# GEM3D/pressurePoissonSolver

Hardware: AMD Instinct MI355X
Metric: V-cycle lattice-site updates/sec, 512^3 3D Poisson (higher is better)
Workload: dtype f64; 1 GPU; apps/3d/steady-equivalent: 512^3 uniform, 4096 patches of 32^3, 5 levels, V(1,1), smoother=rbgs, Dirichlet, f ~ U(-1,1) splitmix64(0x5EED + patch id); workload_key=3d:u512:p32:rbgs, parallelism=patch-sharded x1 (Morton ranges), exchange=none, levels=5, smoother=rbgs

## Files before the change

include/te_hip.h:

```cpp
#ifndef TE_HIP_H
#define TE_HIP_H
#include <stddef.h>
#include <stdint.h>
#ifdef __cplusplus
extern "C" {
#endif

#define TE_OK 0
#define TE_EINVAL -1
#define TE_EHIP -2
#define TE_ESTATE -3
#define TE_EIO -4
#define TE_EUNSUPPORTED -5
#define TE_ENOMEM -6

typedef struct te_mesh te_mesh;
typedef struct te_hier te_hier;
typedef struct te_gmg  te_gmg;
typedef struct te_vec  te_vec;

const char *te_last_error(void);
const char *te_version(void);

int te_mesh_read(const char *path, int dim, te_mesh **out);
// ... 104 lines not shown
                double tol, int *iterations, double *rel_resid);
int te_gmg_release_workspace(te_gmg *g);

int te_prolong_quadratic(te_gmg *g, int fine_level, const te_vec *coarse, te_vec *fine);
int te_fmg(te_gmg *g, const te_cycle_opts *o, const te_vec *f, const te_vec *bdata, te_vec *u, int cycles, double *rel_resid);

int te_patch_indicator(te_gmg *g, int level, const te_vec *u, double *out_host);
int te_vec_regrid(te_gmg *src, const te_vec *u_src, te_gmg *dst, te_vec *u_dst);
int te_faces_regrid(te_gmg *src, const te_vec *U_src, te_gmg *dst, te_vec *U_dst);

int te_gmg_set_option(te_gmg *g, const char *name, const char *value);

enum { TE_SLABS_STENCIL = 0, TE_SLABS_SWEEP = 1 };
int te_gmg_slab_count(const te_gmg *g, int level, int kind, int *zs);

typedef int (*te_exchange_fn)(void *user, int tag, const double *send, double *recv, int npeers,
                              const int32_t *peers, const int64_t *send_off,
                              const int64_t *send_cnt, const int64_t *recv_off,
                              const int64_t *recv_cnt, void *stream);
int te_gmg_set_exchange(te_gmg *g, te_exchange_fn fn, void *user);
int te_rccl_unique_id(const char *libpath, char *id128);
int te_gmg_use_rccl(te_gmg *g, const char *libpath, const char *id128, int rank, int nranks);
typedef int (*te_allreduce_fn)(void *user, double *vals, int n, int op);
int te_gmg_set_allreduce(te_gmg *g, te_allreduce_fn fn, void *user);
int te_gmg_verify_schedule(te_gmg *g, const te_cycle_opts *o);
int te_gmg_autotune(te_gmg *g, const te_cycle_opts *o, int reps, double *best_ms, char *report, int report_len);
int te_gmg_use_push(te_gmg *g, int enable);
int te_gmg_push_failed(te_gmg *g);

int te_gmg_set_patch_bcgs(te_gmg *g, double tol, int max_it);
// ... 56 lines not shown
```

pressurepoissonsolver_amd/capi.py:

```python
import ctypes as C
import os

import numpy as np

_HERE = os.path.dirname(os.path.abspath(__file__))
LIB_PATH = os.environ.get("TE_HIP_LIB_PATH") or os.path.join(_HERE, "libte_hip.so")


class TeError(RuntimeError):

    def __init__(self, code, msg):
        super().__init__(f"te_hip error {code}: {msg}")
        self.code = code


class TeLibraryMissing(ImportError):
    pass


TE_OK, TE_EINVAL, TE_EHIP, TE_ESTATE, TE_EIO, TE_EUNSUPPORTED, TE_ENOMEM = 0, -1, -2, -3, -4, -5, -6
SMOOTH_PATCH_SOLVE, SMOOTH_JACOBI, SMOOTH_RBGS, SMOOTH_PATCH_BCGS = 0, 1, 2, 3
PROBLEM_TRIG, PROBLEM_GAUSS, PROBLEM_RANDOM = 0, 1, 2
SCHUR_PREC_NONE, SCHUR_PREC_CHEB = 0, 1
INTERP_DIRECT, INTERP_LINEAR = 0, 1
# ... 93 lines not shown
    "te_prolong_add": (_I, [_P, _I, _P, _P]),
    "te_prolong_linear_add": (_I, [_P, _I, _P, _P]),
    "te_prolong_quadratic": (_I, [_P, _I, _P, _P]),
    "te_boundary_restrict": (_I, [_P, _I, _P, _P]),
    "te_fmg": (_I, [_P, _P, _P, _P, _P, _I, _PD]),
    "te_patch_indicator": (_I, [_P, _I, _P, _P]),
    "te_vec_regrid": (_I, [_P, _P, _P, _P]),
    "te_faces_regrid": (_I, [_P, _P, _P, _P]),
    "te_gmg_set_interpolator": (_I, [_P, _I]),
    "te_gmg_interpolator": (_I, [_P]),
    "te_vcycle": (_I, [_P, C.POINTER(CycleOpts), _P, _P]),
    "te_bicgstab": (_I, [_P, C.POINTER(CycleOpts), _P, _P, _I, _D, C.POINTER(_I), _PD]),
    "te_gmg_release_workspace": (_I, [_P]),
    "te_gmg_set_option": (_I, [_P, C.c_char_p, C.c_char_p]),
    "te_gmg_slab_count": (_I, [_P, _I, _I, _P]),
    "te_gmg_set_exchange": (_I, [_P, EXCHANGE_FN, _P]),
    "te_rccl_unique_id": (_I, [C.c_char_p, C.c_char_p]),
    "te_gmg_use_rccl": (_I, [_P, C.c_char_p, C.c_char_p, _I, _I]),
    "te_gmg_set_allreduce": (_I, [_P, ALLREDUCE_FN, _P]),
    "te_gmg_verify_schedule": (_I, [_P, C.POINTER(CycleOpts)]),
    "te_gmg_autotune": (_I, [_P, C.POINTER(CycleOpts), _I, _PD, C.c_char_p, _I]),
    "te_gmg_comm_info": (_I, [_P, C.POINTER(_I), C.POINTER(_I)]),
    "te_gmg_use_push": (_I, [_P, _I]),
    "te_gmg_push_failed": (_I, [_P]),
    "te_gmg_set_patch_bcgs": (_I, [_P, _D, _I]),
    "te_gmg_patch_bcgs_iterations": (_I, [_P, _I, _P]),
    "te_gmg_exchange_selftest": (_I, [_P, _I]),
    "te_gmg_watchdog_selftest": (_I, [_P, _D]),
    "te_gmg_setup_ms": (_I, [_P, _PD, _I]),
    "te_gmg_profile": (_I, [_P, _I]),
# ... 478 lines not shown
        return its[:n_local]

    def comm_info(self):
        a, b = C.c_int(), C.c_int()
        check(lib().te_gmg_comm_info(self.h, C.byref(a), C.byref(b)))
        return a.value, b.value

    def set_option(self, name, value="1"):
        check(lib().te_gmg_set_option(self.h, name.encode(), None if value is None else str(value).encode()))

    def slab_count(self, level, kind=0):
        zs = C.c_int()
        check(lib().te_gmg_slab_count(self.h, level, kind, C.byref(zs)))
        return zs.value

    def release_workspace(self):
        check(lib().te_gmg_release_workspace(self.h))

    def set_allreduce(self, fn):
        def cb(user, vals, n, op):
            try:
                out = fn([vals[i] for i in range(n)], op)
                for i in range(n):
                    vals[i] = out[i]
                return 0
            except Exception:
                import traceback
                traceback.print_exc()
                return 1
        self._ar = ALLREDUCE_FN(cb)
# ... 84 lines not shown
```

pressurepoissonsolver_amd/csrc/gmg_core.hip:

```cpp
#include "gmg_internal.hpp"

namespace tei
{
const char *kclassName[KC_COUNT] = {"stencil_apply", "stencil_resid", "stencil_jacobi", "stencil_rbgs",
                                    "cf_ghost", "restrict", "prolong_add", "patch_rhs", "dst_axis",
                                    "vecop", "reduce", "pack", "exchange", "stencil_rbgs_zero", "resid_restrict", "patch_solve_mfma", "stencil_rbgs_prolong",
                                    "stencil_rbgs_slabs", "stencil_slabs", "patch_solve_3pass", "rbgs_zero_resid_restrict",
                                    "restrict_fixup", "rbgs_resweep_prolong", "rbgs_zero_resid_restrict_faces",
                                    "rbgs_resweep_prolong_fcorr", "rbgs_zero_resid_restrict_faces_fcorr", "fcorr_gather", "patch_solve_mfma_faces",
                                    "bicg_update", "bicg_s", "bicg_p", "stencil_apply_dot", "patch_bcgs", "gradient", "divergence", "project", "prolong_linear", "prolong_quadratic", "boundary_restrict",
                                    "indicator", "regrid", "regrid_faces",
                                    "apply_coef", "resid_coef", "jacobi_coef", "rbgs_coef", "faces_restrict"};
const char *optName[O_COUNT] = {"TE_2D_SIMPLE", "TE_2D_NO_MFMA", "TE_2D_NO_PF", "TE_2D_NO_MR_FUSE", "TE_2D_TPB", "TE_NO_FUSE2", "TE_NO_FUSE3",
                                "TE_NO_FUSE3_CF", "TE_NO_CFP", "TE_NO_XF", "TE_NO_FCORR", "TE_NO_FCORR_CF", "TE_NO_OVERLAP",
                                "TE_OVERLAP_MIN", "TE_NO_PS_FACES", "TE_PS_MODE", "TE_PS_SLOW", "TE_RBGS_NOSLAB", "TE_ZS_FORCE", "TE_NO_ZS8",
                                "TE_RESWEEP_V", "TE_EXCHANGE_TIMEOUT", "TE_NO_VERIFY", "TE_RCCL_LOOPBACK", "TE_NO_BICG_FUSE", "TE_POST_EXCHANGE", "TE_REPL_BLOCKS", "TE_PACK_FACES", "TE_OVERLAP_MODE", "TE_PUSH_TIMEOUT", "TE_NO_BICG_XF", "TE_PUSH_FAULT", "TE_2D_NO_FOLD", "TE_2D_NO_SYM", "TE_PUSH_NONFATAL", "TE_PS_NO_HALF", "TE_PS_HALF_MAX", "TE_NO_RS6_CF", "TE_NO_RS6_FIXUP", "TE_SCHUR_FULL", "TE_ZS_PIN"};

void drainEvents(te_gmg *g)
{
	if (g->ev_used == 0) return;
	(void) hipStreamSynchronize(g->stream);
	for (size_t i = 0; i < g->ev_used; i++) {
		float ms = 0;
		if (g->ev_pool[i].valid && hipEventElapsedTime(&ms, g->ev_pool[i].a, g->ev_pool[i].b) == hipSuccess) {
			g->calls[g->ev_pool[i].kc]++;
			g->total_ms[g->ev_pool[i].kc] += ms;
		}
	}
	g->ev_used = 0;
}

// ... 46 lines not shown
	L->prolong_fusable = T.prolong_fusable, L->prolong_fusable_cf = T.prolong_fusable_cf, L->has_copy = T.has_copy;
	L->repl_up = T.repl_up, L->repl_direct = T.repl_direct, L->post_exchange_free = T.post_exchange_free;

	const size_t P1 = (size_t) std::max(T.P, 1), nf = T.nf;
	const bool   fused3d = (D == 3 && T.fuse2_ok && T.P > 0);
	if ((rc = L->send_faces.upload(T.send_faces)) || (rc = L->sendbuf.alloc((size_t) std::max(T.nremote, 1) * nf))
	    || (rc = L->f6off.upload(T.f6off)) || (rc = L->order.upload(T.order)))
		return rc;
	if (D == 3 && ((rc = L->xfbuf[0].alloc(P1 * 2 * nf)) || (rc = L->xfbuf[1].alloc(P1 * 2 * nf)) || (rc = L->f6buf.alloc(P1 * 6 * nf))))
		return rc;
	if (fused3d && li > 0) {
		if ((rc = L->fcorr.alloc((size_t) T.P * 4 * nf))) return rc;
		HIPCHK(hipMemset(L->fcorr.p, 0, sizeof(double) * L->fcorr.n));
	}
	if (fused3d && (rc = L->rs6.alloc((size_t) T.P * 6 * nf / 4))) return rc;
	if ((rc = L->geom_starts.upload(T.geom_starts)) || (rc = L->geom_h.upload(T.geom_h)) || (rc = L->node_ids.upload(T.node_ids))
	    || (rc = L->cellvol.upload(T.cellvol)) || (rc = L->face_kind_patch.upload(T.face_kind_patch))
	    || (rc = L->face_kind.upload(T.face_kind)) || (rc = L->face_src.upload(T.face_src)) || (rc = L->face_kadj.upload(T.face_kadj))
	    || (rc = L->rh2.upload(T.rh2)) || (rc = L->cf_desc.upload(T.cf_desc)) || (rc = L->cf_slots.upload(T.cf_slots))
	    || (rc = L->ghost.alloc((size_t) std::max(T.nslots, 1) * nf)))
		return rc;
	if ((rc = L->matfrag.upload(T.matfrag)) || (rc = L->matsym.upload(T.matsym)) || (rc = L->matsT.upload(T.matsT))
	    || (rc = L->psinv.upload(T.psinv)) || (rc = L->psitab.upload(T.psitab)) || (rc = L->ps_list.upload(T.ps_list))
	    || (rc = L->mat2sym.upload(T.mat2sym)) || (rc = L->ps2_list.upload(T.ps2_list))
	    || (rc = L->corr.alloc(P1 * 2 * D * nf)) || (rc = L->plan.upload(T.plan)) || (rc = L->mats.upload(T.mats))
	    || (rc = L->lam.upload(T.lam)) || (rc = L->zero_mode.upload(T.zero_mode)))
		return rc;
	if (T.coarser
	    && ((D == 2 && T.fuse2_ok && (rc = L->e4buf.alloc(P1 * 4 * n))) || (rc = L->slot_parent.upload(T.slot_parent))
	        || (rc = L->slot_orth.upload(T.slot_orth)) || (rc = L->bc_desc.upload(T.bc_desc)) || (rc = L->cbase.upload(T.cbase))
	        || (rc = L->parent.upload(T.parent)) || (rc = L->orth.upload(T.orth)) || (rc = L->child.upload(T.child))
	        || (rc = L->copy.upload(T.copy)) || (rc = L->up_desc.upload(T.up_desc)) || (rc = L->down_desc.upload(T.down_desc))
	        || (rc = L->up_off.upload(T.up_off)) || (rc = L->down_off.upload(T.down_off))
	        || (rc = L->upbuf.alloc((size_t) std::max<int64_t>(T.up_total, 1)))
	        || (rc = L->downbuf.alloc((size_t) std::max<int64_t>(T.down_total, 1)))))
		return rc;
	g->levels.push_back(std::move(L));
	return TE_OK;
}

int newVec(te_gmg *g, int level, te_vec **out)
{
	LevelHost &L = *g->levels[level];
	auto       v = new te_vec;
	v->g         = g;
// ... 484 lines not shown
}

int te_gmg_slab_count(const te_gmg *g, int level, int kind, int *zs)
{
	return guarded([&]() -> int {
			if (!g || !zs || level < 0 || level >= (int) g->levels.size() || (kind != TE_SLABS_STENCIL && kind != TE_SLABS_SWEEP))
				return te::fail(TE_EINVAL, "te_gmg_slab_count: bad argument");
			const LevelHost &L = *g->levels[level];
			if (L.dim != 3)
				*zs = 1;
			else
				*zs = kind == TE_SLABS_STENCIL ? stencilSlabCount(L.n, L.P, slabSwitches(g)) : rbgsSlabCount(L.n, L.P, slabSwitches(g));
			return TE_OK;
	});
}
}
```

pressurepoissonsolver_amd/csrc/gmg_cycle.hip:

```cpp
#include "gmg_internal.hpp"

namespace tei
{
int smoothOnce(te_gmg *g, int level, const te_vec *f, te_vec *u, int smoother, double omega, bool zero_guess = false, bool faces_only = false)
{
	if (g->coef_on) return coefSmoothOnce(g, level, f, u, smoother, omega);
	LevelHost &L = *g->levels[level];
	int        rc;
	const bool xfok = (L.dim == 3 && g->in_cycle);
	switch (smoother) {
		case TE_SMOOTH_PATCH_SOLVE: {
			bool swapped = false;
			rc           = patchSolve(g, L, f->d, u->d, {zero_guess, nullptr, faces_only}, &swapped);
			if (rc == TE_OK && swapped) swapData(u, L.t.get());
			return rc;
		}
		case TE_SMOOTH_JACOBI:
			L.xf_valid_for = nullptr;
			rc = launchStencil<MODE_JACOBI>(g, L, u->d, f->d, L.t->d, omega);
			if (rc) return rc;
			swapData(u, L.t.get());
			return TE_OK;
		case TE_SMOOTH_RBGS:
			rc = launchRbgs(g, L, u->d, f->d, L.t->d, zero_guess, nullptr, xfok ? xfFor(L, u->d) : nullptr,
			                xfok ? L.xfbuf[L.xf_cur ^ 1].p : nullptr);
			if (rc) return rc;
			if (xfok) xfProduced(L, L.t->d);
			swapData(u, L.t.get());
			return TE_OK;
		case TE_SMOOTH_PATCH_BCGS:
			L.xf_valid_for = nullptr;
			return patchBcgs2d(g, L, f->d, u->d, L.t->d);
		default: return te::fail(TE_EINVAL, "te_smooth: unknown smoother");
	}
}

struct CycleScope {
	te_gmg *g;
	void    forget() const { for (auto &L : g->levels) L->xf_valid_for = nullptr, L->ps_faces = false; }
	explicit CycleScope(te_gmg *g_) : g(g_)
	{
		forget();
		g->in_cycle = !g->cfg.has(O_NO_XF);
	}
	~CycleScope()
	{
		g->in_cycle = false;
		forget();
	}
};

int visit(te_gmg *g, const te_cycle_opts *o, int l, const te_vec *f, te_vec *u, bool u_zero)
{
	const int  nl       = (int) g->levels.size();
	const bool coarsest = (l == nl - 1);
	LevelHost &L        = *g->levels[l];
	int        rc;
	g->cur_level        = l;
	const bool drct = g->interp == TE_INTERP_DIRECT;
	const double *fcorr_in = (L.f_has_corr && L.fcorr.p) ? L.fcorr.p : nullptr;
	L.f_has_corr           = false;
	const Fold2DHost fold_in = L.fold_pending;
	L.fold_pending           = Fold2DHost();
	if (fold_in.fine && coarsest) return te::fail(TE_ESTATE, "te_vcycle: folded ghost terms without a reader");
	const PendingRhs *pend = (l == 0) ? g->pending_rhs : nullptr;
	if (l == 0) g->pending_rhs = nullptr;
	auto formRhs = [&]() -> int {
		if (!pend) return TE_OK;
		const PendingRhs &r = *pend;
		pend                = nullptr;
		if (r.n2 == 0 || g->recording) return TE_OK;
		Timed      t(g, r.kind == 1 ? KC_BICG_S : KC_BICG_P, r.n2 * 2);
		const dim3 grid(gridFor(r.n2, 256, 1 << 30));
// ... 8 lines not shown
	};
	auto       materialise = [&]() -> int {
        if (!u_zero) return TE_OK;
        u_zero         = false;
        L.xf_valid_for = nullptr;
        return vecop<VOP_SET>(u, nullptr, nullptr, 0.0, 0.0, 0.0);
	};
	const double *pending_prolong = nullptr;
	bool          u_unstored      = false;
	int           next_sweeps     = 0;
	auto smooth = [&](int sweeps, bool at_coarsest, bool final_call = false) -> int {
		int sm = o->smoother;
		if (at_coarsest && o->exact_coarse && L.P_global == 1) sm = TE_SMOOTH_PATCH_SOLVE;
		for (int i = 0; i < sweeps; i++) {
			int r;
			if (pending_prolong) {
				const double *c = pending_prolong;
				pending_prolong = nullptr;
				const bool last = final_call && i == sweeps - 1 && !(l == 0 && g->keep_final_xf);
				if (sm == TE_SMOOTH_PATCH_SOLVE) {
					bool swapped = false;
					if ((r = patchSolve(g, L, f->d, u->d, {false, c, false, !last}, &swapped))) return r;
					if (swapped) swapData(u, L.t.get());
					continue;
				}
				double *xo = last ? nullptr : L.xfbuf[L.xf_cur ^ 1].p;
				if (u_unstored) {
					u_unstored = false;
					if ((r = resweepProlong(g, L, f->d, L.t->d, c, xo, fcorr_in))) return r;
				} else if ((r = launchRbgs(g, L, u->d, f->d, L.t->d, false, c, xfFor(L, u->d), xo))) {
					return r;
				}
				if (xo)
					xfProduced(L, L.t->d);
				else
					L.xf_valid_for = nullptr;
				swapData(u, L.t.get());
				continue;
			}
			if (u_zero && ((L.dim == 3 && (sm == TE_SMOOTH_RBGS || sm == TE_SMOOTH_PATCH_SOLVE)) || (L.lds2d && sm == TE_SMOOTH_RBGS)
			               || (L.dim == 2 && sm == TE_SMOOTH_PATCH_SOLVE))) {
				u_zero = false;
				r      = smoothOnce(g, l, f, u, sm, o->omega, true);
			} else {
// ... 83 lines not shown
		if ((rc = smoothOnce(g, l, f, u, TE_SMOOTH_PATCH_SOLVE, o->omega, true, faces_only))) return rc;
		if ((rc = interfaceResidRestrict(g, L, u->d, xfFor(L, u->d), C.f->d, C.f->n))) return rc;
		have_coarse_f = true;
	} else if (o->fuse >= 2 && u_zero && o->pre_sweeps == 1 && o->smoother == TE_SMOOTH_PATCH_SOLVE && ps2dResidFusable(g, L) && !fold_in.fine) {
		if ((rc = formRhs())) return rc;
		u_zero = false;
		if ((rc = smoothOnce(g, l, f, u, TE_SMOOTH_PATCH_SOLVE, o->omega, true))) return rc;
		if ((rc = interfaceResidRestrict2d(g, L, u->d, C.f->d, C.f->n))) return rc;
		have_coarse_f = true;
	} else if (fcorr_in || fold_in.fine) {
		return te::fail(TE_ESTATE, "te_vcycle: exported ghost terms without a reader");
	} else if ((rc = formRhs()) || (rc = smooth(o->pre_sweeps, false))) {
		return rc;
	}
	next_sweeps = (o->cycle_type == 1) ? o->mid_sweeps : o->post_sweeps;
	if ((rc = descend())) return rc;
	if (o->cycle_type == 1) {
		if ((rc = smooth(o->mid_sweeps, false))) return rc;
		next_sweeps = o->post_sweeps;
		if ((rc = descend())) return rc;
	}
	return smooth(o->post_sweeps, false, true);
}

static uint64_t mix64(uint64_t h, uint64_t v)
{
	h ^= v + 0x9E3779B97F4A7C15ull + (h << 6) + (h >> 2);
	h *= 0xBF58476D1CE4E5B9ull;
	return h ^ (h >> 31);
}

// ... 466 lines not shown
```

pressurepoissonsolver_amd/csrc/gmg_fused3d.hip:

```cpp
#include "gmg_ghosts3d.hpp"

namespace tei
{
template <int N>
int zeroSweepResidN(te_gmg *g, LevelHost &L, const double *f, double *out, double *coarse, double *xf_out, bool store_u,
                    double *fcorr_out, const double *fcorr_in, const PendingRhs *fs)
{
	RestrictDst rd = restrictDst(L, coarse);
	const bool export_rs6 = L.rs6.p && !store_u
	                        && (fcorr_out ? (L.prolong_fusable || !g->cfg.has(O_NO_RS6_CF))
	                                      : (L.Pc > 0 || L.n_up > 0) && !fcorr_in && !g->cfg.has(O_NO_RS6_FIXUP));
	rd.rs6                = export_rs6 ? L.rs6.p : nullptr;
	int rc;
	if (L.P > 0) {
		Timed      t(g, store_u ? KC_ZERO_RESID : (fcorr_in ? KC_ZERO_RESID_FACES_FCORR : KC_ZERO_RESID_FACES), (size_t) L.P * L.nc, true);
		if (!store_u) L.f6_tab = L.f6off.p != nullptr && !g->cfg.has(O_PACK_FACES);
		LevelDev   D = L.dev();
		const dim3 grid = slabGrid(L.P), blk(Tile3<N>::TPB);
		if (store_u) {
			D.xf_out = xf_out;
			launchT(t, (k_rbgs_zero_resid3d<N, true>), grid, blk, 0, g->stream, D, f, out, rd, FSrc());
		} else {
			D.f6_out = L.f6buf.p;
			D.fcorr  = fcorr_in;
// ... 35 lines not shown
	} else if (L.P > 0) {
		Timed    t(g, KC_FIXUP, (size_t) L.P * 6 * L.nf);
		LevelDev D = L.dev();
		if (store_u)
			D.xf = xf_out;
		else
			D.f6 = L.f6buf.p;
		hipLaunchKernelGGL((k_restrict_fixup3d<N, false>), dim3(L.P), dim3(256), 0, g->stream, D, out, rd);
	}
	if ((rc = shipRestricted<N>(g, L, coarse))) return rc;
	HIPCHK(hipGetLastError());
	return TE_OK;
}

template <int N>
int resweepProlongN(te_gmg *g, LevelHost &L, const double *f, double *out, const double *prolong_from, double *xf_out, const double *fcorr_in)
{
	ProlongSrc ps      = prolongSrc(L, prolong_from);
	const bool refined = L.ncf > 0 || L.has_copy;
	const int v = resweepVariant(fcorr_in != nullptr, refined, L.index, (size_t) L.P * L.nc * sizeof(double), g->resweep_pin);
	if (!v) return te::fail(TE_ESTATE, "resweepProlong: exported ghost terms on a refined level");
	auto launch = [&](LevelDev D) {
		if (D.count == 0) return;
		Timed t(g, fcorr_in ? KC_RESWEEP_FCORR : KC_RESWEEP, (size_t) D.count * L.nc, true);
		D.f6    = L.f6buf.p;
		D.fcorr = fcorr_in;
		const dim3 grid = slabGrid(D.count), blk(Tile3<N>::TPB);
		if (refined) {
			if (v == 59)
				launchT(t, (k_rbgs_resweep_prolong3d<N, 59, false, true>), grid, blk, 0, g->stream, D, f, out, ps);
			else
				launchT(t, (k_rbgs_resweep_prolong3d<N, 27, false, true>), grid, blk, 0, g->stream, D, f, out, ps);
		} else if (v == 3) {
			launchT(t, (k_rbgs_resweep_prolong3d<N, 3, true>), grid, blk, 0, g->stream, D, f, out, ps);
// ... 10 lines not shown
		ps.gorth      = L.slot_orth.p;
		L.ghost_has_v = false;
		LevelDev D    = L.dev();
		D.xf_out      = xf_out;
		launch(D);
		HIPCHK(hipGetLastError());
		return TE_OK;
	}
	int rc = withGhosts<N>(g, L, {nullptr, L.f6buf.p, &ps}, launch, nullptr, xf_out);
	if (rc) return rc;
	HIPCHK(hipGetLastError());
	return TE_OK;
}

int resweepProlong(te_gmg *g, LevelHost &L, const double *f, double *out, const double *prolong_from, double *xf_out,
                   const double *fcorr_in)
{
	if (L.dim == 2) return resweepProlong2d(g, L, f, out, prolong_from);
	return dispatchN(L.n, [&](auto n) { return resweepProlongN<decltype(n)::value>(g, L, f, out, prolong_from, xf_out, fcorr_in); });
}

template <int N> int interfaceResidRestrictN(te_gmg *g, LevelHost &L, const double *u, const double *xf, double *coarse, size_t coarse_n)
{
	RestrictDst rd = restrictDst(L, coarse);
	int rc;
	if ((rc = prepareGhosts<N>(g, L, {u, L.ps_faces ? L.f6buf.p : nullptr}))) return rc;
	{
		Timed t(g, KC_VECOP, coarse_n);
		if (L.repl_up && L.repl_direct && !g->cfg.has(O_REPL_BLOCKS) && !L.tx_direct.empty()) {
			if (L.tx_direct.send_cnt[0] > 0)
				HIPCHK(hipMemsetAsync(coarse + L.tx_direct.send_off[0], 0, sizeof(double) * (size_t) L.tx_direct.send_cnt[0], g->stream));
		} else
			HIPCHK(hipMemsetAsync(coarse, 0, sizeof(double) * coarse_n, g->stream));
		if (L.n_up > 0) HIPCHK(hipMemsetAsync(L.upbuf.p, 0, sizeof(double) * L.upbuf.n, g->stream));
// ... 29 lines not shown
```

pressurepoissonsolver_amd/csrc/gmg_internal.hpp:

```cpp
#pragma once
#include "capi_common.hpp"
#include "dispatch.hpp"
#include "level_tables.hpp"
#include <hip/hip_ext.h>
#include <rccl/rccl.h>
#include "kernels3d.hpp"
#include "march3d.hpp"
#include "kernels2d.hpp"
#include "patchsolve32.hpp"
#include "patchsolve32_sym.hpp"
#include "patchsolve16.hpp"
#include "initkernels.hpp"
#include "bckernels.hpp"
#include "pushkernels.hpp"
#include <algorithm>
#include <array>
#include <atomic>
#include <chrono>
#include <cmath>
#include <cstdio>
#include <cstring>
#include <dlfcn.h>
#include <map>
#include <memory>
// ... 36 lines not shown
	KC_PS_MFMA_FACES,
	KC_BICG_UPDATE, KC_BICG_S, KC_BICG_P, KC_APPLY_DOT,
	KC_PATCH_BCGS,
	KC_GRADIENT, KC_DIVERGENCE, KC_PROJECT,
	KC_PROLONG_LINEAR,
	KC_PROLONG_QUADRATIC, KC_BOUNDARY_RESTRICT,
	KC_INDICATOR, KC_REGRID,
	KC_FACE_REGRID,
	KC_APPLY_COEF, KC_RESID_COEF, KC_JACOBI_COEF, KC_RBGS_COEF, KC_FACES_RESTRICT, KC_COUNT
};
extern const char *kclassName[KC_COUNT];

enum Opt : int {
	O_2D_SIMPLE, O_2D_NO_MFMA, O_2D_NO_PF, O_2D_NO_MR_FUSE, O_2D_TPB, O_NO_FUSE2, O_NO_FUSE3, O_NO_FUSE3_CF, O_NO_CFP, O_NO_XF,
	O_NO_FCORR, O_NO_FCORR_CF, O_NO_OVERLAP, O_OVERLAP_MIN, O_NO_PS_FACES, O_PS_MODE, O_PS_SLOW, O_RBGS_NOSLAB,
	O_ZS_FORCE, O_NO_ZS8, O_RESWEEP_V, O_EXCHANGE_TIMEOUT, O_NO_VERIFY, O_RCCL_LOOPBACK, O_NO_BICG_FUSE, O_POST_EXCHANGE, O_REPL_BLOCKS, O_PACK_FACES, O_OVERLAP_MODE, O_PUSH_TIMEOUT, O_NO_BICG_XF, O_PUSH_FAULT, O_2D_NO_FOLD, O_2D_NO_SYM, O_PUSH_NONFATAL, O_PS_NO_HALF, O_PS_HALF_MAX, O_NO_RS6_CF, O_NO_RS6_FIXUP, O_SCHUR_FULL, O_ZS_PIN, O_COUNT
};
extern const char *optName[O_COUNT];
inline bool optStructural(int o) { return o == O_2D_SIMPLE || o == O_NO_CFP || o == O_2D_NO_MR_FUSE || o == O_NO_OVERLAP || o == O_EXCHANGE_TIMEOUT; }
struct Cfg {
	bool        on[O_COUNT] = {};
	std::string val[O_COUNT];
	void        set(int o, const char *v)
	{
		on[o]  = v != nullptr;
		val[o] = v ? v : "";
	}
	void fromEnv();
	bool        has(int o) const { return on[o]; }
	const char *str(int o) const { return on[o] ? val[o].c_str() : nullptr; }
	int         num(int o, int dflt) const { return on[o] ? atoi(val[o].c_str()) : dflt; }
// ... 57 lines not shown
	bool   fuse2_ok = false;
	size_t nc = 0, nf = 0;
	DevBuf<int32_t> face_kind, face_src;
	DevBuf<int32_t> face_kind_patch;
	DevBuf<double>  face_kadj, rh2, ghost;
	int             nslots = 0;
	int             ncf = 0;
	DevBuf<int32_t> cf_desc, cf_slots;
	ExPlan          fx;
	int             nremote = 0;
	DevBuf<int32_t> send_faces;
	DevBuf<double>  sendbuf;
	int             Pc = 0;
	DevBuf<int32_t> parent, orth, child, copy;
	DevBuf<int64_t> cbase;
	ExPlan          tx_up, tx_down;
	int             n_up = 0, n_down = 0;
	bool            repl_up = false;
	DevBuf<int32_t> bc_desc;
	DevBuf<int32_t> up_desc, down_desc;
	DevBuf<int64_t> up_off, down_off;
	DevBuf<double>  upbuf, downbuf;
	DevBuf<int32_t> plan, zero_mode;
	DevBuf<int32_t> bcgs_its;
	DevBuf<double>  mats, lam, corr;
	DevBuf<double>  matsT;
	DevBuf<double>  matfrag;
	DevBuf<double>  matsym;
	DevBuf<double>  psinv;
	DevBuf<int32_t> psitab;
// ... 379 lines not shown
		if (idx < 0) return;
		auto &w = g->wd;
		std::lock_guard<std::mutex> lk(w.mu);
		w.batch     = -1;
		auto &sl    = w.slot[idx % te_gmg::Watchdog::RING];
		sl.recorded = (hipEventRecord(sl.ev, g->stream) == hipSuccess);
	}
};

template <int MODE> int launchStencil(te_gmg *g, LevelHost &L, const double *u, const double *f, double *out, double omega,
                                      RestrictDst rd = RestrictDst(), const double *xf_in = nullptr, int redmode = RED_NONE,
                                      const double *red_a = nullptr, int *red_items = nullptr, bool patch_op = false);
extern template int launchStencil<MODE_APPLY>(te_gmg *, LevelHost &, const double *, const double *, double *, double, RestrictDst, const double *, int, const double *, int *, bool);
extern template int launchStencil<MODE_RESID>(te_gmg *, LevelHost &, const double *, const double *, double *, double, RestrictDst, const double *, int, const double *, int *, bool);
extern template int launchStencil<MODE_JACOBI>(te_gmg *, LevelHost &, const double *, const double *, double *, double, RestrictDst, const double *, int, const double *, int *, bool);
int resweepProlong(te_gmg *g, LevelHost &L, const double *f, double *out, const double *prolong_from, double *xf_out, const double *fcorr_in);
int interfaceResidRestrict(te_gmg *g, LevelHost &L, const double *u, const double *xf, double *coarse, size_t coarse_n);
int zeroSweepResid(te_gmg *g, LevelHost &L, const double *f, double *out, double *coarse, double *xf_out, bool store_u,
                   double *fcorr_out = nullptr, const double *fcorr_in = nullptr, const PendingRhs *fs = nullptr,
                   const Fold2DHost *fold_in = nullptr, bool skip_fixup = false);
int launchRbgs(te_gmg *g, LevelHost &L, const double *u, const double *f, double *out, bool zero_guess = false,
               const double *prolong_from = nullptr, const double *xf_in = nullptr, double *xf_out = nullptr);
int residRestrict(te_gmg *g, LevelHost &L, const double *u, const double *f, double *coarse, const double *xf_in = nullptr);
bool psOnePass(const te_gmg *g, const LevelHost &L);
int  psSymCount(const te_gmg *g, const LevelHost &L);
bool psAllSym32(const te_gmg *g, const LevelHost &L);
struct PatchSolveOpts {
	bool          zero_guess   = false;
	const double *prolong_from = nullptr;
	bool          faces_only   = false;
	bool          export_xf    = true;
// ... 136 lines not shown
```

pressurepoissonsolver_amd/csrc/level_tables.cpp:

```cpp
#include "level_tables.hpp"
#include "capi_common.hpp"
#include "table_layout.hpp"
#include <algorithm>
#include <array>
#include <cmath>
#include <map>
#include <tuple>

using namespace te;

namespace tei
{
namespace
{
using PeerItems = std::vector<std::pair<int, int64_t>>;

void transformMatrix(int type, int n, double *m)
{
	static const double oi[6] = {0.0, 0.5, 0.5, 1.0, 0.5, 0.5}, oj[6] = {0.5, 0.0, 0.5, 0.5, 1.0, 0.5};
	for (int i = 0; i < n; i++) {
		for (int j = 0; j < n; j++) {
			const double x = M_PI / n * ((i + oi[type]) * (j + oj[type]));
			m[i * n + j]   = type < 3 ? cos(x) : sin(x);
		}
// ... 504 lines not shown
		T.tx_up   = mergePlan(ups, downs);
		T.tx_down = mergePlan(downs, ups);
	}
	if (T.prolong_fusable && D == 3) {
		const int64_t nn = (int64_t) n * n, nnn = nn * n, hh = n / 2;
		auto          base = [&](int p) {
            const int o = orth[p];
            return (int64_t) parent[p] * nnn + ((o & 1) ? hh : 0) + n * ((o & 2) ? hh : 0) + nn * ((o & 4) ? hh : 0);
		};
		T.cbase.assign((size_t) std::max(P, 1) * 7, -1);
		for (int p = 0; p < P; p++) {
			T.cbase[(size_t) p * 7] = base(p);
			for (int s = 0; s < 6; s++)
				if (T.face_kind[(size_t) p * 6 + s] == FACE_LOCAL) T.cbase[(size_t) p * 7 + 1 + s] = base(T.face_src[(size_t) p * 6 + s]);
		}
	}
	return TE_OK;
}

int boundaryRestrictTable(const Level &lv, const Level &cv, LevelTables &T)
{
	const int            D = lv.dim, NS = 2 * D, NQ = 1 << (D - 1);
	std::vector<int32_t> cb;
	const int            ncb = te::bfaceIndex(cv, cb);
	T.brestrict.assign((size_t) ncb * 5, -1);
	for (int p = 0; p < lv.P; p++) {
		const int pc = T.parent[p], o = T.orth[p];
		for (int s = 0; s < NS; s++) {
			const int fb = T.bface[(size_t) p * NS + s];
			if (fb < 0) continue;
// ... 55 lines not shown
```

pressurepoissonsolver_amd/csrc/level_tables.hpp:

```cpp
#pragma once
#include "mesh.hpp"
#include <cstddef>
#include <cstdint>
#include <vector>

namespace tei
{
struct ExPlan {
	std::vector<int32_t> peers;
	std::vector<int64_t> send_off, send_cnt, recv_off, recv_cnt;
	bool empty() const { return peers.empty(); }
};

struct LevelBuildOpts {
	bool simple_2d = false, no_cfp = false, no_mr_fuse_2d = false;
};

struct LevelTables {
	int    dim = 3, n = 0, P = 0, P_global = 0;
	bool   replicated = false, gathered = false;
	size_t nc = 0, nf = 0;
	ExPlan               fx;
	int                  nremote = 0;
	std::vector<int32_t> send_faces, f6off;
	std::vector<int32_t> face_kind, face_kind_patch, face_src, cf_desc, cf_slots, order, node_ids;
	std::vector<double>  face_kadj, rh2, cellvol, patch_vol, geom_starts, geom_h;
	int                  nslots = 0, ncf = 0, n_int = 0, n_bnd = 0;
	bool                 lds2d = false, fuse2d = false, fuse2_ok = false;
	std::vector<int32_t> plan, zero_mode, psitab, ps_list, ps2_list;
	std::vector<double>  mats, lam, matsT, matfrag, matsym, psinv, mat2sym;
	bool                 sym_ok = false;
	int                  n_pure = 0, n_pure2 = 0;
	bool                 coarser = false;
	int                  Pc = 0, n_up = 0, n_down = 0;
	std::vector<int32_t> parent, orth, child, copy, up_desc, down_desc, bc_desc, slot_parent, slot_orth;
	std::vector<int64_t> up_off, down_off, cbase;
	int64_t              up_total = 0, down_total = 0;
	ExPlan               tx_up, tx_down, tx_direct;
	bool prolong_fusable = false, prolong_fusable_cf = false, has_copy = false, repl_up = false, repl_direct = false,
	     post_exchange_free = false;
	int                  nif = -1;
	std::vector<int32_t> if_own, if_start, if_contrib;
	int                  nbf = 0;
	std::vector<int32_t> bface;
	std::vector<int32_t> brestrict;
};

int computeLevelTables(const te::Hierarchy &H, int li, const LevelBuildOpts &o, LevelTables &out);

}
```

pressurepoissonsolver_amd/csrc/march3d.hpp:

```cpp
#pragma once
#include "kernels3d.hpp"
#include <type_traits>

namespace te
{
template <bool NT> __device__ __forceinline__ double2 ldStream(const double2 *p)
{
	if (NT) {
		double2 v;
		v.x = __builtin_nontemporal_load(&p->x);
		v.y = __builtin_nontemporal_load(&p->y);
		return v;
	}
	return *p;
}
template <bool NT> __device__ __forceinline__ void stStream(double2 *p, double2 v)
{
	if (NT) {
		__builtin_nontemporal_store(v.x, &p->x);
		__builtin_nontemporal_store(v.y, &p->y);
	} else
		*p = v;
}
__device__ __forceinline__ double2 takeRegs(const double2 &src)
// ... 265 lines not shown
	if (RED != RED_NONE) {
		__syncthreads();
		blockReduce2(acc0, acc1);
		if (tid == 0) {
			red.partial[2 * ((size_t) red.base + work)]     = acc0;
			red.partial[2 * ((size_t) red.base + work) + 1] = acc1;
		}
	}
}

struct ProlongSrc {
	const int32_t *parent, *orth;
	const double  *coarse;
	const int32_t *gparent = nullptr, *gorth = nullptr;
	const int64_t *cbase = nullptr;
};
template <int N> __device__ __forceinline__ const double *coarseOctantSlot(const ProlongSrc &ps, int slot)
{
	constexpr int NN = N * N, NNN = N * N * N, H = N / 2;
	const int     o = ps.gorth[slot];
	return ps.coarse + (size_t) ps.gparent[slot] * NNN + ((o & 1) ? H : 0) + N * ((o & 2) ? H : 0) + NN * ((o & 4) ? H : 0);
}
template <int N> __device__ __forceinline__ const double *coarseOctant(const ProlongSrc &ps, int p)
{
	constexpr int NN = N * N, NNN = N * N * N, H = N / 2;
	const int     o = ps.orth[p];
	return ps.coarse + (size_t) ps.parent[p] * NNN + ((o & 1) ? H : 0) + N * ((o & 2) ? H : 0) + NN * ((o & 4) ? H : 0);
}

template <int N> __device__ __forceinline__ double coarseAtCell(const ProlongSrc &ps, int p, int cell)
{
// ... 1029 lines not shown
		const int cx0 = (X == 0) ? 0 : 1, cx1 = (X == H - 1) ? 2 : 1;
		dix[0][0] = cx0 + 3 * cy0, dix[0][1] = cx1 + 3 * cy0, dix[1][0] = cx0 + 3 * cy1, dix[1][1] = cx1 + 3 * cy1;
	}

	static_assert(!CFP || !FCORR, "the exported ghost terms are for uniformly refined levels");
	const bool    cpo  = CFP && ps.orth[pid] < 0;
	const double *yown = cpo ? ps.coarse + (size_t) ps.parent[pid] * NNN : nullptr;
	const double *cown = cpo ? yown : coarseOctant<N>(ps, pid), *chalo = cown, *cbot = cown, *ctop = cown;
	double        shalo = 0.0, sbot = 0.0, stop = 0.0;
	const int     cq = X + N * Yp;
	bool          cpb = false, cpt = false;
	const double *ybot = nullptr, *ytop = nullptr;
	int           hsh = 1;
	if (tid < 4 * N) {
		const int side = tid / N, t = tid % N;
		if (fk[side] == FACE_LOCAL) {
			if (CFP && ps.orth[fs[side]] < 0) {
				const int nbr = (side == 0) ? t * N + (N - 1) : (side == 1 ? t * N : (side == 2 ? (N - 1) * N + t : t));
				chalo = ps.coarse + (size_t) ps.parent[fs[side]] * NNN + nbr;
				hsh   = 0;
			} else {
				const double *cn = coarseOctant<N>(ps, fs[side]);
				const int     cx = (side == 0) ? H - 1 : (side == 1 ? 0 : t / 2);
				const int     cy = (side == 2) ? H - 1 : (side == 3 ? 0 : t / 2);
				chalo = cn + cx + N * cy;
			}
			shalo = 1.0;
		} else if (!CFP && fk[side] == FACE_GHOST && ps.gparent) {
			const double *cn = coarseOctantSlot<N>(ps, fs[side]);
			const int     cx = (side == 0) ? H - 1 : (side == 1 ? 0 : t / 2);
			const int     cy = (side == 2) ? H - 1 : (side == 3 ? 0 : t / 2);
			chalo = cn + cx + N * cy;
			shalo = 1.0;
		}
	}
// ... 215 lines not shown
			relaxCell<N, 0, (0 + ZPAR) & 1, false>(tz, idiag, cz9, lds, ldo, dix, act, rhx, rhy, rhz, uc, um, un, f0);
			relaxCell<N, 1, (1 + ZPAR) & 1, false>(tz, idiag, cz9, lds, ldo, dix, act, rhx, rhy, rhz, uc, um, un, f0);
		}
		if (z > 0) {
			const int cz9 = cz9of(z - 1);
			relaxCell<N, 0, (1 + 0 + 1 - ZPAR) & 1, false, false>(tm, idiag, cz9, lds, ldo, dix, act, rhx, rhy, rhz, um, umm, uc, fm);
			relaxCell<N, 1, (1 + 1 + 1 - ZPAR) & 1, false, false>(tm, idiag, cz9, lds, ldo, dix, act, rhx, rhy, rhz, um, umm, uc, fm);
			if (act) {
				stStream<NTS>(op2 + (z - 1) * NP + q[0], um[0]);
				stStream<NTS>(op2 + (z - 1) * NP + q[1], um[1]);
				if (L.xf_out) {
					double *xo = L.xf_out + (size_t) pid * 2 * NN + N * (z - 1) + 2 * Yp;
					if (X == 0) *reinterpret_cast<double2 *>(xo) = double2{um[0].x, um[1].x};
					if (X == H - 1) *reinterpret_cast<double2 *>(xo + NN) = double2{um[0].y, um[1].y};
				}
			}
		}
#pragma unroll
		for (int k = 0; k < 2; k++) {
			umm[k] = um[k];
			um[k]  = uc[k];
			uc[k]  = un[k];
			un[k]  = un2[k];
			r1[k]  = r2[k];
			r2[k]  = r3[k];
		}
		bz = (bz == 2) ? 0 : bz + 1;
	};
	constexpr int U = RING;
	using NotLast = std::integral_constant<bool, false>;
// ... 28 lines not shown
```

Measured before the change: 142.5 billion lattice-site updates/s.

## Export compact coarse x-face planes during prolong resweep for finer-level halo reads

During the final post-smoothing resweep of a 3D coarse level, the kernel now also writes selected x-face/midplane columns of each patch into a compact per-group buffer (cxp). When the next finer level prolongs from that coarse solution, x-side halo reads of neighbouring coarse octants use this packed buffer via precomputed offsets (cxoff) instead of strided gathers from the full coarse array. The goal is fewer scattered global loads in the prolong-fused smoother, at the cost of extra stores, an added buffer, host-side validity tracking across levels, and an opt-out flag. Counters and an API to query export/read counts are included.

```diff
diff --git a/include/te_hip.h b/include/te_hip.h
--- a/include/te_hip.h
+++ b/include/te_hip.h
@@ -142,6 +142,8 @@
 enum { TE_SLABS_STENCIL = 0, TE_SLABS_SWEEP = 1 };
 int te_gmg_slab_count(const te_gmg *g, int level, int kind, int *zs);
 
+int te_gmg_cxp_counts(const te_gmg *g, int level, int64_t *exports, int64_t *reads);
+
 typedef int (*te_exchange_fn)(void *user, int tag, const double *send, double *recv, int npeers,
                               const int32_t *peers, const int64_t *send_off,
                               const int64_t *send_cnt, const int64_t *recv_off,
diff --git a/pressurepoissonsolver_amd/capi.py b/pressurepoissonsolver_amd/capi.py
--- a/pressurepoissonsolver_amd/capi.py
+++ b/pressurepoissonsolver_amd/capi.py
@@ -131,6 +131,7 @@
     "te_gmg_release_workspace": (_I, [_P]),
     "te_gmg_set_option": (_I, [_P, C.c_char_p, C.c_char_p]),
     "te_gmg_slab_count": (_I, [_P, _I, _I, _P]),
+    "te_gmg_cxp_counts": (_I, [_P, _I, _P, _P]),
     "te_gmg_set_exchange": (_I, [_P, EXCHANGE_FN, _P]),
     "te_rccl_unique_id": (_I, [C.c_char_p, C.c_char_p]),
     "te_gmg_use_rccl": (_I, [_P, C.c_char_p, C.c_char_p, _I, _I]),
@@ -639,6 +640,11 @@
         check(lib().te_gmg_slab_count(self.h, level, kind, C.byref(zs)))
         return zs.value
 
+    def cxp_counts(self, level):
+        ex, rd = C.c_int64(), C.c_int64()
+        check(lib().te_gmg_cxp_counts(self.h, level, C.byref(ex), C.byref(rd)))
+        return ex.value, rd.value
+
     def release_workspace(self):
         check(lib().te_gmg_release_workspace(self.h))
 
diff --git a/pressurepoissonsolver_amd/csrc/gmg_core.hip b/pressurepoissonsolver_amd/csrc/gmg_core.hip
--- a/pressurepoissonsolver_amd/csrc/gmg_core.hip
+++ b/pressurepoissonsolver_amd/csrc/gmg_core.hip
@@ -14,7 +14,7 @@
 const char *optName[O_COUNT] = {"TE_2D_SIMPLE", "TE_2D_NO_MFMA", "TE_2D_NO_PF", "TE_2D_NO_MR_FUSE", "TE_2D_TPB", "TE_NO_FUSE2", "TE_NO_FUSE3",
                                 "TE_NO_FUSE3_CF", "TE_NO_CFP", "TE_NO_XF", "TE_NO_FCORR", "TE_NO_FCORR_CF", "TE_NO_OVERLAP",
                                 "TE_OVERLAP_MIN", "TE_NO_PS_FACES", "TE_PS_MODE", "TE_PS_SLOW", "TE_RBGS_NOSLAB", "TE_ZS_FORCE", "TE_NO_ZS8",
-                                "TE_RESWEEP_V", "TE_EXCHANGE_TIMEOUT", "TE_NO_VERIFY", "TE_RCCL_LOOPBACK", "TE_NO_BICG_FUSE", "TE_POST_EXCHANGE", "TE_REPL_BLOCKS", "TE_PACK_FACES", "TE_OVERLAP_MODE", "TE_PUSH_TIMEOUT", "TE_NO_BICG_XF", "TE_PUSH_FAULT", "TE_2D_NO_FOLD", "TE_2D_NO_SYM", "TE_PUSH_NONFATAL", "TE_PS_NO_HALF", "TE_PS_HALF_MAX", "TE_NO_RS6_CF", "TE_NO_RS6_FIXUP", "TE_SCHUR_FULL", "TE_ZS_PIN"};
+                                "TE_RESWEEP_V", "TE_EXCHANGE_TIMEOUT", "TE_NO_VERIFY", "TE_RCCL_LOOPBACK", "TE_NO_BICG_FUSE", "TE_POST_EXCHANGE", "TE_REPL_BLOCKS", "TE_PACK_FACES", "TE_OVERLAP_MODE", "TE_PUSH_TIMEOUT", "TE_NO_BICG_XF", "TE_PUSH_FAULT", "TE_2D_NO_FOLD", "TE_2D_NO_SYM", "TE_PUSH_NONFATAL", "TE_PS_NO_HALF", "TE_PS_HALF_MAX", "TE_NO_RS6_CF", "TE_NO_RS6_FIXUP", "TE_SCHUR_FULL", "TE_NO_CXP", "TE_ZS_PIN"};
 
 void drainEvents(te_gmg *g)
 {
@@ -91,6 +91,9 @@
 		HIPCHK(hipMemset(L->fcorr.p, 0, sizeof(double) * L->fcorr.n));
 	}
 	if (fused3d && (rc = L->rs6.alloc((size_t) T.P * 6 * nf / 4))) return rc;
+	if (D == 3 && li > 0 && T.P > 0 && n >= 8 && g->levels[li - 1]->cxoff.p && g->levels[li - 1]->fuse2_ok
+	    && (rc = L->cxp.alloc((size_t) ((T.P + n / 4 - 1) / (n / 4)) * n * nf)))
+		return rc;
 	if ((rc = L->geom_starts.upload(T.geom_starts)) || (rc = L->geom_h.upload(T.geom_h)) || (rc = L->node_ids.upload(T.node_ids))
 	    || (rc = L->cellvol.upload(T.cellvol)) || (rc = L->face_kind_patch.upload(T.face_kind_patch))
 	    || (rc = L->face_kind.upload(T.face_kind)) || (rc = L->face_src.upload(T.face_src)) || (rc = L->face_kadj.upload(T.face_kadj))
@@ -105,7 +108,7 @@
 		return rc;
 	if (T.coarser
 	    && ((D == 2 && T.fuse2_ok && (rc = L->e4buf.alloc(P1 * 4 * n))) || (rc = L->slot_parent.upload(T.slot_parent))
-	        || (rc = L->slot_orth.upload(T.slot_orth)) || (rc = L->bc_desc.upload(T.bc_desc)) || (rc = L->cbase.upload(T.cbase))
+	        || (rc = L->slot_orth.upload(T.slot_orth)) || (rc = L->bc_desc.upload(T.bc_desc)) || (rc = L->cbase.upload(T.cbase)) || (rc = L->cxoff.upload(T.cxoff))
 	        || (rc = L->parent.upload(T.parent)) || (rc = L->orth.upload(T.orth)) || (rc = L->child.upload(T.child))
 	        || (rc = L->copy.upload(T.copy)) || (rc = L->up_desc.upload(T.up_desc)) || (rc = L->down_desc.upload(T.down_desc))
 	        || (rc = L->up_off.upload(T.up_off)) || (rc = L->down_off.upload(T.down_off))
@@ -620,4 +623,15 @@
 			return TE_OK;
 	});
 }
-}
+
+int te_gmg_cxp_counts(const te_gmg *g, int level, int64_t *exports, int64_t *reads)
+{
+	return guarded([&]() -> int {
+			if (!g || !exports || !reads || level < 0 || level >= (int) g->levels.size())
+				return te::fail(TE_EINVAL, "te_gmg_cxp_counts: bad argument");
+			*exports = g->levels[level]->cxp_exports;
+			*reads   = g->levels[level]->cxp_reads;
+			return TE_OK;
+	});
+}
+}
diff --git a/pressurepoissonsolver_amd/csrc/gmg_cycle.hip b/pressurepoissonsolver_amd/csrc/gmg_cycle.hip
--- a/pressurepoissonsolver_amd/csrc/gmg_cycle.hip
+++ b/pressurepoissonsolver_amd/csrc/gmg_cycle.hip
@@ -37,7 +37,7 @@
 
 struct CycleScope {
 	te_gmg *g;
-	void    forget() const { for (auto &L : g->levels) L->xf_valid_for = nullptr, L->ps_faces = false; }
+	void    forget() const { for (auto &L : g->levels) L->xf_valid_for = nullptr, L->cxp_valid_for = nullptr, L->wants_cxp = false, L->ps_faces = false; }
 	explicit CycleScope(te_gmg *g_) : g(g_)
 	{
 		forget();
@@ -57,6 +57,7 @@
 	LevelHost &L        = *g->levels[l];
 	int        rc;
 	g->cur_level        = l;
+	L.cxp_valid_for     = nullptr;
 	const bool drct = g->interp == TE_INTERP_DIRECT;
 	const double *fcorr_in = (L.f_has_corr && L.fcorr.p) ? L.fcorr.p : nullptr;
 	L.f_has_corr           = false;
@@ -95,6 +96,7 @@
 		if (at_coarsest && o->exact_coarse && L.P_global == 1) sm = TE_SMOOTH_PATCH_SOLVE;
 		for (int i = 0; i < sweeps; i++) {
 			int r;
+			L.cxp_valid_for = nullptr;
 			if (pending_prolong) {
 				const double *c = pending_prolong;
 				pending_prolong = nullptr;
@@ -108,7 +110,8 @@
 				double *xo = last ? nullptr : L.xfbuf[L.xf_cur ^ 1].p;
 				if (u_unstored) {
 					u_unstored = false;
-					if ((r = resweepProlong(g, L, f->d, L.t->d, c, xo, fcorr_in))) return r;
+					const bool cx = final_call && i == sweeps - 1 && l > 0 && g->levels[l - 1]->wants_cxp;
+					if ((r = resweepProlong(g, L, f->d, L.t->d, c, xo, fcorr_in, cx))) return r;
 				} else if ((r = launchRbgs(g, L, u->d, f->d, L.t->d, false, c, xfFor(L, u->d), xo))) {
 					return r;
 				}
@@ -222,7 +225,10 @@
 		return rc;
 	}
 	next_sweeps = (o->cycle_type == 1) ? o->mid_sweeps : o->post_sweeps;
-	if ((rc = descend())) return rc;
+	L.wants_cxp = u_unstored && L.dim == 3 && L.prolong_fusable;
+	rc          = descend();
+	L.wants_cxp = false;
+	if (rc) return rc;
 	if (o->cycle_type == 1) {
 		if ((rc = smooth(o->mid_sweeps, false))) return rc;
 		next_sweeps = o->post_sweeps;
diff --git a/pressurepoissonsolver_amd/csrc/gmg_fused3d.hip b/pressurepoissonsolver_amd/csrc/gmg_fused3d.hip
--- a/pressurepoissonsolver_amd/csrc/gmg_fused3d.hip
+++ b/pressurepoissonsolver_amd/csrc/gmg_fused3d.hip
@@ -73,10 +73,24 @@
 }
 
 template <int N>
-int resweepProlongN(te_gmg *g, LevelHost &L, const double *f, double *out, const double *prolong_from, double *xf_out, const double *fcorr_in)
+int resweepProlongN(te_gmg *g, LevelHost &L, const double *f, double *out, const double *prolong_from, double *xf_out, const double *fcorr_in,
+                    bool export_cxp)
 {
 	ProlongSrc ps      = prolongSrc(L, prolong_from);
 	const bool refined = L.ncf > 0 || L.has_copy;
+	if (N >= 8 && !refined && !g->cfg.has(O_NO_CXP)) {
+		LevelHost *C = L.index + 1 < (int) g->levels.size() ? g->levels[L.index + 1].get() : nullptr;
+		if (C && C->cxp.p && L.cxoff.p && C->cxp_valid_for == prolong_from) {
+			ps.cxp   = C->cxp.p;
+			ps.cxoff = L.cxoff.p;
+			if (!g->recording && L.P > 0) L.cxp_reads++;
+		}
+		if (export_cxp && L.cxp.p) {
+			ps.cxp_out = L.cxp.p;
+			if (!g->recording && L.P > 0) L.cxp_exports++;
+		}
+	}
+	L.cxp_valid_for = ps.cxp_out ? out : nullptr;
 	const int v = resweepVariant(fcorr_in != nullptr, refined, L.index, (size_t) L.P * L.nc * sizeof(double), g->resweep_pin);
 	if (!v) return te::fail(TE_ESTATE, "resweepProlong: exported ghost terms on a refined level");
 	auto launch = [&](LevelDev D) {
@@ -117,10 +131,12 @@
 }
 
 int resweepProlong(te_gmg *g, LevelHost &L, const double *f, double *out, const double *prolong_from, double *xf_out,
-                   const double *fcorr_in)
+                   const double *fcorr_in, bool export_cxp)
 {
 	if (L.dim == 2) return resweepProlong2d(g, L, f, out, prolong_from);
-	return dispatchN(L.n, [&](auto n) { return resweepProlongN<decltype(n)::value>(g, L, f, out, prolong_from, xf_out, fcorr_in); });
+	return dispatchN(L.n, [&](auto n) {
+		return resweepProlongN<decltype(n)::value>(g, L, f, out, prolong_from, xf_out, fcorr_in, export_cxp);
+	});
 }
 
 template <int N> int interfaceResidRestrictN(te_gmg *g, LevelHost &L, const double *u, const double *xf, double *coarse, size_t coarse_n)
diff --git a/pressurepoissonsolver_amd/csrc/gmg_internal.hpp b/pressurepoissonsolver_amd/csrc/gmg_internal.hpp
--- a/pressurepoissonsolver_amd/csrc/gmg_internal.hpp
+++ b/pressurepoissonsolver_amd/csrc/gmg_internal.hpp
@@ -74,7 +74,7 @@
 enum Opt : int {
 	O_2D_SIMPLE, O_2D_NO_MFMA, O_2D_NO_PF, O_2D_NO_MR_FUSE, O_2D_TPB, O_NO_FUSE2, O_NO_FUSE3, O_NO_FUSE3_CF, O_NO_CFP, O_NO_XF,
 	O_NO_FCORR, O_NO_FCORR_CF, O_NO_OVERLAP, O_OVERLAP_MIN, O_NO_PS_FACES, O_PS_MODE, O_PS_SLOW, O_RBGS_NOSLAB,
-	O_ZS_FORCE, O_NO_ZS8, O_RESWEEP_V, O_EXCHANGE_TIMEOUT, O_NO_VERIFY, O_RCCL_LOOPBACK, O_NO_BICG_FUSE, O_POST_EXCHANGE, O_REPL_BLOCKS, O_PACK_FACES, O_OVERLAP_MODE, O_PUSH_TIMEOUT, O_NO_BICG_XF, O_PUSH_FAULT, O_2D_NO_FOLD, O_2D_NO_SYM, O_PUSH_NONFATAL, O_PS_NO_HALF, O_PS_HALF_MAX, O_NO_RS6_CF, O_NO_RS6_FIXUP, O_SCHUR_FULL, O_ZS_PIN, O_COUNT
+	O_ZS_FORCE, O_NO_ZS8, O_RESWEEP_V, O_EXCHANGE_TIMEOUT, O_NO_VERIFY, O_RCCL_LOOPBACK, O_NO_BICG_FUSE, O_POST_EXCHANGE, O_REPL_BLOCKS, O_PACK_FACES, O_OVERLAP_MODE, O_PUSH_TIMEOUT, O_NO_BICG_XF, O_PUSH_FAULT, O_2D_NO_FOLD, O_2D_NO_SYM, O_PUSH_NONFATAL, O_PS_NO_HALF, O_PS_HALF_MAX, O_NO_RS6_CF, O_NO_RS6_FIXUP, O_SCHUR_FULL, O_NO_CXP, O_ZS_PIN, O_COUNT
 };
 extern const char *optName[O_COUNT];
 inline bool optStructural(int o) { return o == O_2D_SIMPLE || o == O_NO_CFP || o == O_2D_NO_MR_FUSE || o == O_NO_OVERLAP || o == O_EXCHANGE_TIMEOUT; }
@@ -162,6 +162,11 @@
 	int             Pc = 0;
 	DevBuf<int32_t> parent, orth, child, copy;
 	DevBuf<int64_t> cbase;
+	DevBuf<double>  cxp;
+	const double   *cxp_valid_for = nullptr;
+	DevBuf<int64_t> cxoff;
+	bool            wants_cxp = false;
+	int64_t         cxp_exports = 0, cxp_reads = 0;
 	ExPlan          tx_up, tx_down;
 	int             n_up = 0, n_down = 0;
 	bool            repl_up = false;
@@ -571,7 +576,8 @@
 extern template int launchStencil<MODE_APPLY>(te_gmg *, LevelHost &, const double *, const double *, double *, double, RestrictDst, const double *, int, const double *, int *, bool);
 extern template int launchStencil<MODE_RESID>(te_gmg *, LevelHost &, const double *, const double *, double *, double, RestrictDst, const double *, int, const double *, int *, bool);
 extern template int launchStencil<MODE_JACOBI>(te_gmg *, LevelHost &, const double *, const double *, double *, double, RestrictDst, const double *, int, const double *, int *, bool);
-int resweepProlong(te_gmg *g, LevelHost &L, const double *f, double *out, const double *prolong_from, double *xf_out, const double *fcorr_in);
+int resweepProlong(te_gmg *g, LevelHost &L, const double *f, double *out, const double *prolong_from, double *xf_out, const double *fcorr_in,
+                   bool export_cxp = false);
 int interfaceResidRestrict(te_gmg *g, LevelHost &L, const double *u, const double *xf, double *coarse, size_t coarse_n);
 int zeroSweepResid(te_gmg *g, LevelHost &L, const double *f, double *out, double *coarse, double *xf_out, bool store_u,
                    double *fcorr_out = nullptr, const double *fcorr_in = nullptr, const PendingRhs *fs = nullptr,
diff --git a/pressurepoissonsolver_amd/csrc/level_tables.cpp b/pressurepoissonsolver_amd/csrc/level_tables.cpp
--- a/pressurepoissonsolver_amd/csrc/level_tables.cpp
+++ b/pressurepoissonsolver_amd/csrc/level_tables.cpp
@@ -542,6 +542,17 @@
 			for (int s = 0; s < 6; s++)
 				if (T.face_kind[(size_t) p * 6 + s] == FACE_LOCAL) T.cbase[(size_t) p * 7 + 1 + s] = base(T.face_src[(size_t) p * 6 + s]);
 		}
+		if (n >= 8 && n % 4 == 0 && !T.repl_up) {
+			const int64_t grp = n / 4;
+			T.cxoff.assign((size_t) std::max(P, 1) * 2, -1);
+			for (int p = 0; p < P; p++)
+				for (int s = 0; s < 2; s++) {
+					if (T.face_kind[(size_t) p * 6 + s] != FACE_LOCAL) continue;
+					const int     q = T.face_src[(size_t) p * 6 + s], o = orth[q];
+					const int64_t c = parent[q], j = (s == 0 ? 1 : 0) + ((o & 1) ? 2 : 0);
+					T.cxoff[(size_t) p * 2 + s] = (c / grp) * nnn + (c % grp) * 4 * n + nn * ((o & 4) ? hh : 0) + n * j + ((o & 2) ? hh : 0);
+				}
+		}
 	}
 	return TE_OK;
 }
diff --git a/pressurepoissonsolver_amd/csrc/level_tables.hpp b/pressurepoissonsolver_amd/csrc/level_tables.hpp
--- a/pressurepoissonsolver_amd/csrc/level_tables.hpp
+++ b/pressurepoissonsolver_amd/csrc/level_tables.hpp
@@ -34,7 +34,7 @@
 	bool                 coarser = false;
 	int                  Pc = 0, n_up = 0, n_down = 0;
 	std::vector<int32_t> parent, orth, child, copy, up_desc, down_desc, bc_desc, slot_parent, slot_orth;
-	std::vector<int64_t> up_off, down_off, cbase;
+	std::vector<int64_t> up_off, down_off, cbase, cxoff;
 	int64_t              up_total = 0, down_total = 0;
 	ExPlan               tx_up, tx_down, tx_direct;
 	bool prolong_fusable = false, prolong_fusable_cf = false, has_copy = false, repl_up = false, repl_direct = false,
diff --git a/pressurepoissonsolver_amd/csrc/march3d.hpp b/pressurepoissonsolver_amd/csrc/march3d.hpp
--- a/pressurepoissonsolver_amd/csrc/march3d.hpp
+++ b/pressurepoissonsolver_amd/csrc/march3d.hpp
@@ -303,7 +303,15 @@
 	const double  *coarse;
 	const int32_t *gparent = nullptr, *gorth = nullptr;
 	const int64_t *cbase = nullptr;
+	const double  *cxp     = nullptr;
+	const int64_t *cxoff   = nullptr;
+	double        *cxp_out = nullptr;
 };
+template <int N> __host__ __device__ __forceinline__ size_t cxpBase(int p)
+{
+	constexpr int G = N / 4;
+	return (size_t) (p / G) * (N * N * N) + (size_t) (p % G) * (4 * N);
+}
 template <int N> __device__ __forceinline__ const double *coarseOctantSlot(const ProlongSrc &ps, int slot)
 {
 	constexpr int NN = N * N, NNN = N * N * N, H = N / 2;
@@ -1363,11 +1371,14 @@
 	int           hsh = 1;
 	if (tid < 4 * N) {
 		const int side = tid / N, t = tid % N;
+		const int64_t cxo = (!CFP && N >= 8 && side < 2 && ps.cxoff) ? ps.cxoff[(size_t) pid * 2 + side] : -1;
 		if (fk[side] == FACE_LOCAL) {
 			if (CFP && ps.orth[fs[side]] < 0) {
 				const int nbr = (side == 0) ? t * N + (N - 1) : (side == 1 ? t * N : (side == 2 ? (N - 1) * N + t : t));
 				chalo = ps.coarse + (size_t) ps.parent[fs[side]] * NNN + nbr;
 				hsh   = 0;
+			} else if (cxo >= 0) {
+				chalo = ps.cxp + cxo + t / 2;
 			} else {
 				const double *cn = coarseOctant<N>(ps, fs[side]);
 				const int     cx = (side == 0) ? H - 1 : (side == 1 ? 0 : t / 2);
@@ -1613,6 +1624,17 @@
 					if (X == 0) *reinterpret_cast<double2 *>(xo) = double2{um[0].x, um[1].x};
 					if (X == H - 1) *reinterpret_cast<double2 *>(xo + NN) = double2{um[0].y, um[1].y};
 				}
+				if constexpr (!CFP && N >= 8) {
+					if (ps.cxp_out) {
+						unsigned qq = (unsigned) q[0];
+						asm volatile("" : "+v"(qq));
+						const unsigned xq = qq & (unsigned) (H - 1);
+						const bool     hi = (xq == H / 2 - 1) | (xq == H - 1);
+						const unsigned j  = (xq >= H / 2 ? 2u : 0u) + (hi ? 1u : 0u);
+						double2       *cp = reinterpret_cast<double2 *>(ps.cxp_out + cxpBase<N>(pid) + NN * (z - 1) + qq / (unsigned) H);
+						if (hi | (xq == 0) | (xq == H / 2)) cp[j * H] = hi ? double2{um[0].y, um[1].y} : double2{um[0].x, um[1].x};
+					}
+				}
 			}
 		}
 #pragma unroll
```

Result: no change. 143.0 billion lattice-site updates/s, median of 2 (+0.3%).
